# BDMstudio/audio-cut

Hardware: AMD Instinct MI355X
Metric: audio-seconds processed/sec (separate+detect) per GPU; cut-point index parity (higher is better)
Workload: dtype f32

## Files before the change

### audio_cut_amd/_native.py

```python
from __future__ import annotations

import ctypes as C
import threading
import os
from pathlib import Path
from typing import Optional, Sequence, Tuple

import numpy as np
import torch

_LIB_NAME = "libaudiocut_hip.so"
_lib: Optional[C.CDLL] = None


class NativeError(RuntimeError):
    pass


def library_path() -> Path:
    return Path(__file__).resolve().parent / os.environ.get("AUDIOCUT_HIP_LIBNAME", _LIB_NAME)


def load() -> C.CDLL:
    global _lib
    if _lib is not None:
        return _lib
    path = library_path()
    if not path.exists():
        raise NativeError(f"{path} is missing: build it with `make -C audio_cut_amd/csrc` "
                          f"(there is no CPU fallback for the HIP path)")
    lib = C.CDLL(str(path))
    _declare(lib)
    if lib.ac_abi_version() != 6:
        raise NativeError("libaudiocut_hip.so ABI version mismatch")
    if lib.ac_stereo_abi_version() != 1:
        raise NativeError("libaudiocut_hip.so stereo ABI version mismatch")
    if lib.ac_onset_abi_version() != 1:
        raise NativeError("libaudiocut_hip.so onset ABI version mismatch")
    if lib.ac_beat_abi_version() != 1:
        raise NativeError("libaudiocut_hip.so beat ABI version mismatch")
    if lib.ac_hybrid_abi_version() != 1:
        raise NativeError("libaudiocut_hip.so hybrid ABI version mismatch")
    if lib.ac_export_abi_version() != 1:
        raise NativeError("libaudiocut_hip.so export ABI version mismatch")
    if lib.ac_asr_abi_version() != 1:
        raise NativeError("libaudiocut_hip.so asr ABI version mismatch")
    if lib.ac_profile_abi_version() != 1:
        raise NativeError("libaudiocut_hip.so profile ABI version mismatch")
    if lib.ac_final_abi_version() != 1:
        raise NativeError("libaudiocut_hip.so final-layer ABI version mismatch")
    if lib.ac_load_abi_version() != 1:
        raise NativeError("libaudiocut_hip.so loader ABI version mismatch")
    if lib.ac_pack_abi_version() != 1:
        raise NativeError("libaudiocut_hip.so pack ABI version mismatch")
    _lib = lib
    return lib


_P = C.c_void_p
_I64 = C.c_int64
_I = C.c_int

SIGNATURES = {
    "ac_abi_version": (C.c_int, []),
    "ac_last_error": (C.c_char_p, []),
    "ac_ctx_create": (C.c_int, [_I, C.POINTER(_P)]),
    "ac_ctx_destroy": (C.c_int, [_P]),
    "ac_frame_rms": (C.c_int, [_P, _P, _I64, _I, _I, _I, _P, _I64, _P]),
    "ac_frame_rms_multi": (C.c_int, [_P, _P, _I64, _I, _P, _P, _P, _P, _P]),
    "ac_stft2048_features": (C.c_int, [_P, _P, _I64, _I, _P, _P, _P, _P, _P, _I64, _P]),
    "ac_onset_strength": (C.c_int, [_P, _P, _I64, _P, _I, _I, _I, _P, _P, _P]),
    "ac_tempogram_parts": (C.c_int, [_I64]),
    "ac_tempogram_reduce": (C.c_int, [_P, _P, _I64, _I, _P, _P, _P, _P, _P]),
    "ac_yin_f0": (C.c_int, [_P, _P, _I64, _I, _I, _I, _I, C.c_double, _P, _P, _I64, _P]),
    "ac_moving_meansq_db_f64": (C.c_int, [_P, _P, _I64, _I, _P, _P]),
    "ac_next_leq_scratch": (C.c_int64, [_I64]),
    "ac_next_leq_scan": (C.c_int, [_P, _P, _I64, C.c_double, _P, _P, _P]),
    "ac_window_argmin_f64": (C.c_int, [_P, _P, _I64, _P, _P, _I, _P, _P, _P]),
    "ac_zero_cross_nearest": (C.c_int, [_P, _P, _I64, _P, _I, _I, _P, _P]),
    "ac_quiet_guard_slow": (C.c_int, [_P, _P, _I64, _P, _I, _I, _I, _P, _P, _P]),
    "ac_pause_cut_points": (C.c_int, [_P, _P, _I64, _P, _P, _I, _I, _I, _P, _P, _P]),
    "ac_mdx_stft": (C.c_int, [_P, _P, _I64, _P, _P, _P, _I, _P, _P, _P]),
    "ac_mdx_istft": (C.c_int, [_P, _P, _I, _P, _P, _P]),
    "ac_mdx_assemble_ola": (C.c_int, [_P, _P, _I64, _P, _P, _P, _P, _P, _P, _I, _P, _P, _P]),
    "ac_mdx_chunk_vocal": (C.c_int, [_P, _P, _P, _P, _P, _I, _P, _P]),
    "ac_sum_squares": (C.c_int, [_P, _P, _I64, _P, _I, _P]),
    "ac_window_sum_squares": (C.c_int, [_P, _P, _I64, _P, _P, _I, _P, _P]),
    "ac_conv3x3_f16x3": (C.c_int, [_P, _P, _P, _P, _P, _I, _I, _I, _I, _I, C.c_float, _I, _P, _P, _P]),
    "ac_conv3x3_f16x3_w96": (C.c_int, [_P, _P, _P, _P, _P, _I, _I, _I, _I, _I, C.c_float, _I, _P, _P, _P]),
    "ac_conv3x3_f16x3_s8": (C.c_int, [_P, _P, _P, _P, _P, _I, _I, _I, _I, _I, C.c_float, _I, _P, _P, _P]),
    "ac_conv3x3_f16x3_first": (C.c_int, [_P, _P, _P, _P, _P, _P, _P, _I, _I, _I, _I, _I, _I, C.c_float, _I, _P, C.c_float, C.c_float,
                                         _P, _P]),
    "ac_tdf_linear_f16x3": (C.c_int, [_P, _P, _P, _P, _P, _P, _P, _I64, _I, _I, _I, _I, C.c_float, _P, _P, _P]),
    "ac_tdf_small_fused": (C.c_int, [_P, _P, _P, _P, _P, _P, _P, _P, _P, _I64, _I, _I, _I, _I, _P, _P]),
    "ac_conv1x1_small": (C.c_int, [_P, _P, _P, _P, _P, _I, _I, _I, _I64, _I, _P]),
    "ac_down2x_f16x3": (C.c_int, [_P, _P, _P, _P, _P, _I, _I, _I, _I, _I, C.c_float, _P, _P, _P]),
    "ac_up2x_f16x3": (C.c_int, [_P, _P, _P, _P, _P, _P, _I, _I, _I, _I, _I, C.c_float, _P, _P, _P]),
    "ac_pyin_observe": (C.c_int, [_P, _P, _I64, _I, _I, C.c_double, C.c_double, _I, _I, _P, _P, _P, _P, _P, C.c_double, C.c_double,
                                  _P, _P, _P, _P]),
    "ac_pyin_viterbi": (C.c_int, [_P, _P, _P, _I64, _I, _I, _P, _P, C.c_double, _P, _P, _P, _P]),
    "ac_lpc_formants": (C.c_int, [_P, _P, _I64, _I, _I, _I, C.c_float, _P, _P, _I64, _P]),
    "ac_zero_crossing_rate": (C.c_int, [_P, _P, _I64, _I, _I, _P, _I64, _P]),
    "ac_stft2048_spectral": (C.c_int, [_P, _P, _I64, _I, C.c_double, _P, _P, _I64, _P]),
    "ac_segment_frame_rms": (C.c_int, [_P, _P, _I64, _P, _P, _P, _I, _I, _I, _I, _P, _I64, _P]),
    "ac_segment_sumsq_peak": (C.c_int, [_P, _P, _I64, _P, _P, _I, _P, _P, _P]),
    "ac_local_valley_tiles": (C.c_int, [_I, _I]),
    "ac_local_valley": (C.c_int, [_P, _P, _I64, _P, _I, _I, _I, _P, _P, _P, _P, _P, _P]),
    "ac_resample_poly": (C.c_int, [_P, _P, _I64, _I, _I, _P, _I64, _I64, _P, _I64, _P]),
    "ac_pack_pcm24": (C.c_int, [_P, _P, _I64, _P, _P]),
    "ac_resample_poly_segments": (C.c_int, [_P, _P, _P, _P, _P, _P, _I, _I, _I, _P, _I64, _I64, _P, _I64, _P]),
    "ac_silero_frontend": (C.c_int, [_P, _P, _P, _I, _P, _P, _P, _P, _P, _P, _P, _P, _P, _P, _P, _P, _P]),
    "ac_silero_lstm": (C.c_int, [_P, _P, _P, _P, _I, _P, _P, _P]),
    "ac_silero_out": (C.c_int, [_P, _P, _P, C.c_float, _I, _P, _P]),
    "ac_host_beat_dp": (C.c_int, [_P, _I64, C.c_double, C.c_double, _P, _P]),
}

STEREO_SIGNATURES = {
    "ac_stereo_abi_version": (C.c_int, []),
    "ac_mdx_stft_stereo": (C.c_int, [_P, _P, _I64, _P, _P, _P, _I, _P, _P, _P]),
    "ac_mdx_assemble_ola_stereo": (C.c_int, [_P, _P, _I64, _P, _P, _P, _P, _P, _P, _I, _P, _P, _P, _P, _P]),
    "ac_mdx_chunk_vocal_stereo": (C.c_int, [_P, _P, _I64, _P, _P, _P, _P, _P, _I, _I, _P, _P]),
}


ONSET_SIGNATURES = {
    "ac_onset_abi_version": (C.c_int, []),
    "ac_bar_energy_silence": (C.c_int, [_P, _P, _I64, _P, _P, _I, C.c_double, _P, _P, _P]),
    "ac_segment_pair_energy": (C.c_int, [_P, _P, _P, _I64, _P, _P, _I, _P, _P]),
}

BEAT_SIGNATURES = {
    "ac_beat_abi_version": (C.c_int, []),
    "ac_stft2048_centroid_bandwidth": (C.c_int, [_P, _P, _I64, _I, C.c_double, _P, _P, _I64, _P]),
    "ac_bar_means3": (C.c_int, [_P, _P, _I64, _P, _P, _I64, _P, _P, _I, _P, _P]),
}

HYBRID_SIGNATURES = {
    "ac_hybrid_abi_version": (C.c_int, []),
    "ac_quiet_gate_meansq": (C.c_int, [_P, _P, _I64, _I64, _P, _I, _P, _I64, _P, _P, _P]),
}

EXPORT_SIGNATURES = {
    "ac_export_abi_version": (C.c_int, []),
    "ac_mdx_assemble_pcm24": (C.c_int, [_P, _P, _I64, _I, _P, _P, _P, _P, _P, _P, _I, _P, _P, _P, _I, _P]),
}

ASR_SIGNATURES = {
    "ac_asr_abi_version": (C.c_int, []),
    "ac_resample_poly_pcm16": (C.c_int, [_P, _P, _I64, _I, _I, _P, _I64, _I64, _P, _I64, _P]),
}

PROFILE_SIGNATURES = {
    "ac_profile_abi_version": (C.c_int, []),
    "ac_abs_peak_coverage": (C.c_int, [_P, _P, _I64, C.c_double, C.c_double, _P, _P, _P, _P]),
}
FINAL_SIGNATURES = {
    "ac_final_abi_version": (C.c_int, []),
    "ac_tdf_linear_final_f16x3": (C.c_int, [_P, _P, _P, _P, _P, _P, _P, _P, _P, _P, _I64, _I, _I, _I, _I, _I, C.c_float, _P, _P]),
}
LOAD_SIGNATURES = {
    "ac_load_abi_version": (C.c_int, []),
    "ac_decode_pcm": (C.c_int, [_P, _P, _I64, _I, _I, _I, _P, _I64, _P, _P]),
}
PACK_SIGNATURES = {
    "ac_pack_abi_version": (C.c_int, []),
    "ac_pack_width": (C.c_int, [_I]),
    "ac_pack_out_align": (C.c_int, [_I]),
    "ac_pack_pcm": (C.c_int, [_P, _P, _I64, _I, _I64, _I, _P, _P]),
    "ac_mdx_assemble_pcm": (C.c_int, [_P, _P, _I64, _I, _P, _P, _P, _P, _P, _P, _I, _I, _P, _P, _P, _I, _P]),
}
from .utils.audio_export import WAV_SUBTYPES as PACK_SUBTYPES, subtype_info as pack_subtype


PROFILE_GRID_SAMPLES = 4 * 256 * 2048


def coverage_from(peak: float, count: int, n: int) -> float:
    if int(n) == 0 or float(peak) <= 1e-9:
        return 0.0
    return max(0.0, min(1.0, int(count) / int(n)))


def _declare(lib: C.CDLL) -> None:
    for name, (res, args) in (*SIGNATURES.items(), *STEREO_SIGNATURES.items(), *ONSET_SIGNATURES.items(), *BEAT_SIGNATURES.items(),
                              *HYBRID_SIGNATURES.items(), *EXPORT_SIGNATURES.items(), *ASR_SIGNATURES.items(), *PROFILE_SIGNATURES.items(),
                              *FINAL_SIGNATURES.items(), *LOAD_SIGNATURES.items(), *PACK_SIGNATURES.items()):
        fn = getattr(lib, name)
        fn.restype = res
        fn.argtypes = args


def _check(rc: int) -> None:
    if rc != 0:
        msg = load().ac_last_error()
        raise NativeError(f"libaudiocut_hip call failed ({rc}): {msg.decode() if msg else '?'}")


def _ptr(t: Optional[torch.Tensor]) -> Optional[int]:
    if t is None:
        return None
    if not t.is_contiguous():
        raise NativeError("non-contiguous tensor passed to the HIP ABI")
    return t.data_ptr()


def _stream() -> int:
    return torch.cuda.current_stream().cuda_stream


def _packed(name: str, t: Optional[torch.Tensor], n_bytes: Optional[int]) -> None:
    if t is None or n_bytes is None:
        return
    have = t.numel() * t.element_size()
    if have != n_bytes:
        raise NativeError(f"{name}: the packed weights hold {have} bytes, the shape implies {n_bytes} (see separation/conv_pack.py)")


def _conv3x3_packed_bytes(c_in: int, c_out: int, cob: int, stage: int) -> Optional[int]:
    if c_in <= 0 or c_out <= 0 or c_in % 16 or c_out % cob:
        return None
    return (c_out // cob) * (c_in // stage) * (5 if stage == 16 else 3) * 2 * (cob // 16) * 64 * 8 * 2


def _linear_packed_bytes(n: int, k: int, bn: int) -> Optional[int]:
    if n <= 0 or k <= 0 or (bn == 0 and (n % 96 or k % 32)):
        return None
    n2 = -(-n // bn) * bn if bn else n
    return 2 * n2 * (-(-k // 32) * 32) * 2


class Context:

    def __init__(self, device: str = "cuda:0"):
        if not torch.cuda.is_available():
            raise NativeError("no HIP device visible to PyTorch: the audio-cut HIP path needs a GPU")
        self.device = torch.device(device)
        if self.device.type != "cuda":
            raise NativeError(f"device {device!r} is not a HIP device")
        self.index = self.device.index if self.device.index is not None else torch.cuda.current_device()
        self.device = torch.device("cuda", self.index)
        self.lib = load()
        handle = _P()
        with torch.cuda.device(self.index):
            _check(self.lib.ac_ctx_create(self.index, C.byref(handle)))
        self._h = handle
        self._rs_filters: dict = {}
        self._pf = threading.local()

    def close(self) -> None:
        if getattr(self, "_h", None):
            self.lib.ac_ctx_destroy(self._h)
            self._h = None

    def __del__(self):
        try:
            self.close()
        except Exception:
            pass

    SMALL_UPLOAD_BYTES = 1 << 20

    def to_device(self, arr, dtype=None) -> torch.Tensor:
        t = torch.as_tensor(np.ascontiguousarray(arr))
        if dtype is not None:
            t = t.to(dtype)
        if 0 < t.numel() * t.element_size() <= self.SMALL_UPLOAD_BYTES and not t.is_cuda:
            staged = torch.empty(t.shape, dtype=t.dtype, pin_memory=True)
            staged.copy_(t)
            return staged.to(self.device, non_blocking=True)
# ... 803 lines not shown
            raise NativeError("conv1x1_small expects a contiguous float32 NCHW tensor")
        b, c, h, w = x.shape
        w2 = weight.reshape(weight.shape[0], -1)
        if w2.shape[1] != c or not w2.is_contiguous():
            raise NativeError("conv1x1_small: weight must be [C_out, C_in(,1,1)] contiguous")
        _packed("conv1x1_small (bias)", bias, w2.shape[0] * 4)
        out = torch.empty((b, w2.shape[0], h, w), dtype=torch.float32, device=self.device)
        _check(self.lib.ac_conv1x1_small(self._h, _ptr(x), _ptr(w2), _ptr(bias), _ptr(out), b, c, w2.shape[0], h * w, int(relu), _stream()))
        return out

    def down2x_f16x3(self, x: torch.Tensor, w_packed: torch.Tensor, bias: torch.Tensor, c_out: int, w_unscale: float,
                     in_amax: Optional[torch.Tensor] = None, out_amax: Optional[torch.Tensor] = None) -> torch.Tensor:
        if x.dtype != torch.float32 or x.dim() != 4 or not x.is_contiguous():
            raise NativeError("down2x_f16x3 expects a contiguous float32 NCHW tensor")
        b, c, h, w = x.shape
        _packed("down2x_f16x3", w_packed, _linear_packed_bytes(int(c_out), 4 * c, 96))
        out = torch.empty((b, c_out, h // 2, w // 2), dtype=torch.float32, device=self.device)
        pi, po = self._amax_args(b, in_amax, out_amax, h, h // 2)
        _check(self.lib.ac_down2x_f16x3(self._h, _ptr(x), _ptr(w_packed), _ptr(bias), _ptr(out), b, c, c_out, h, w, float(w_unscale),
                                        pi, po, _stream()))
        return out

    def up2x_f16x3(self, x: torch.Tensor, w_packed: torch.Tensor, bias: torch.Tensor, c_out: int, w_unscale: float,
                   skip: Optional[torch.Tensor] = None, in_amax: Optional[torch.Tensor] = None,
                   out_amax: Optional[torch.Tensor] = None) -> torch.Tensor:
        if x.dtype != torch.float32 or x.dim() != 4 or not x.is_contiguous():
            raise NativeError("up2x_f16x3 expects a contiguous float32 NCHW tensor")
        b, c, h, w = x.shape
        _packed("up2x_f16x3", w_packed, _linear_packed_bytes(4 * int(c_out), c, 96))
        out = torch.empty((b, c_out, 2 * h, 2 * w), dtype=torch.float32, device=self.device)
        if skip is not None and (skip.shape != out.shape or not skip.is_contiguous() or skip.dtype != torch.float32):
            raise NativeError("up2x_f16x3: skip must match the output")
        pi, po = self._amax_args(b, in_amax, out_amax, h, 2 * h)
        _check(self.lib.ac_up2x_f16x3(self._h, _ptr(x), _ptr(w_packed), _ptr(bias), _ptr(skip), _ptr(out), b, c, c_out, h, w,
                                      float(w_unscale), pi, po, _stream()))
        return out

    def sum_squares_parts(self, x: torch.Tensor) -> torch.Tensor:
        self._chk_f32(x)
        hit = self._pf_take("sum_squares_parts", x)
        if hit is not None:
            return hit
        n = x.numel()
        parts = min(1024, max(1, n // 4096))
        buf = torch.empty(parts, dtype=torch.float64, device=self.device)
        _check(self.lib.ac_sum_squares(self._h, _ptr(x), n, _ptr(buf), parts, _stream()))
        return buf

    WINDOW_MEAN_SQUARE_MAX = 8191

    def window_mean_squares(self, x: torch.Tensor, starts, ends) -> np.ndarray:
        self._chk_f32(x)
        a = np.asarray(starts, dtype=np.int64); b = np.asarray(ends, dtype=np.int64)
        n = int(x.numel())
        if a.shape != b.shape or a.ndim != 1:
            raise ValueError("starts / ends must be equally long 1-D sequences")
        if a.size == 0:
            return np.zeros(0, dtype=np.float64)
        if np.any(a < 0) or np.any(b > n) or np.any(b < a) or np.any(b - a > self.WINDOW_MEAN_SQUARE_MAX):
            raise ValueError("windows must lie inside the wave and be at most WINDOW_MEAN_SQUARE_MAX samples long")
        out = torch.empty(a.size, dtype=torch.float64, device=self.device)
        a_dev, b_dev = self.to_device(a), self.to_device(b)
        _check(self.lib.ac_window_sum_squares(self._h, _ptr(x), n, _ptr(a_dev), _ptr(b_dev), int(a.size), _ptr(out), _stream()))
        sums = out.cpu().numpy()
        length = (b - a).astype(np.float64)
        return np.where(length > 0, sums / np.where(length > 0, length, 1.0), 0.0)

    def mean_square(self, x: torch.Tensor) -> float:
        self._chk_f32(x)
        n = x.numel()
        if n == 0:
            return 0.0
        return float(np.sum(self.sum_squares_parts(x).cpu().numpy())) / float(n)


def host_beat_dp(localscore: np.ndarray, period: float, tightness: float):
    lib = load()
    ls = np.ascontiguousarray(localscore, dtype=np.float64)
    n = ls.size
    back = np.empty(n, dtype=np.int64)
    cum = np.zeros(n, dtype=np.float64)
    _check(lib.ac_host_beat_dp(ls.ctypes.data, n, float(period), float(tightness), back.ctypes.data, cum.ctypes.data))
    return back, cum
```

### audio_cut_amd/csrc/ac_mdx.hip

```cpp
#include <math.h>

#include "ac_common.h"
#include "../../include/audiocut_hip_stereo.h"

#define MDX_NFFT 6144
#define MDX_M 3072
#define MDX_HOP 1024
#define MDX_T 256
#define MDX_F 3072
#define MDX_ITEM 261120
#define MDX_TRIM 3072
#define MDX_GEN 254976

__device__ inline float2 cmulf(float2 a, float2 b) { return make_float2(a.x * b.x - a.y * b.y, a.x * b.y + a.y * b.x); }

__device__ inline float2 tw3072(const float2* __restrict__ tw, int q) {
    int k = 2 * q;
    if (k >= MDX_M) { const float2 t = tw[k - MDX_M]; return make_float2(-t.x, -t.y); }
    return tw[k];
}

__device__ float2* fft3072_f32(float2* a, float2* b, const float2* __restrict__ tw) {
    int Ns = 1;
    for (int pass = 0; pass < 5; ++pass) {
        for (int j = threadIdx.x; j < MDX_M / 4; j += 256) {
            const int k = j & (Ns - 1);
            float2 v0 = a[j], v1 = a[j + MDX_M / 4], v2 = a[j + MDX_M / 2], v3 = a[j + 3 * MDX_M / 4];
            if (Ns > 1) {
                const int q = k * (MDX_M / (4 * Ns));
                v1 = cmulf(v1, tw3072(tw, q));
                v2 = cmulf(v2, tw3072(tw, 2 * q));
                v3 = cmulf(v3, tw3072(tw, 3 * q));
            }
            const float2 s02 = make_float2(v0.x + v2.x, v0.y + v2.y), d02 = make_float2(v0.x - v2.x, v0.y - v2.y);
            const float2 s13 = make_float2(v1.x + v3.x, v1.y + v3.y), d13 = make_float2(v1.x - v3.x, v1.y - v3.y);
            const int base = ((j - k) << 2) + k;
            b[base] = make_float2(s02.x + s13.x, s02.y + s13.y);
            b[base + Ns] = make_float2(d02.x + d13.y, d02.y - d13.x);
            b[base + 2 * Ns] = make_float2(s02.x - s13.x, s02.y - s13.y);
            b[base + 3 * Ns] = make_float2(d02.x - d13.y, d02.y + d13.x);
        }
        __syncthreads();
        float2* t = a; a = b; b = t;
        Ns <<= 2;
    }
    {
        const float c3 = -0.5f, s3 = -0.86602540378443864676f;
        for (int j = threadIdx.x; j < MDX_M / 3; j += 256) {
            const int k = j;
            float2 v0 = a[j], v1 = a[j + 1024], v2 = a[j + 2048];
            v1 = cmulf(v1, tw3072(tw, k));
            v2 = cmulf(v2, tw3072(tw, 2 * k));
            const float2 s = make_float2(v1.x + v2.x, v1.y + v2.y);
            const float2 d = make_float2(v1.x - v2.x, v1.y - v2.y);
            const float2 m = make_float2(v0.x + c3 * s.x, v0.y + c3 * s.y);
            const float2 r = make_float2(-s3 * d.y, s3 * d.x);
            b[k] = make_float2(v0.x + s.x, v0.y + s.y);
            b[k + 1024] = make_float2(m.x + r.x, m.y + r.y);
            b[k + 2048] = make_float2(m.x - r.x, m.y - r.y);
        }
        __syncthreads();
        float2* t = a; a = b; b = t;
    }
    return a;
}

template <int CH>
__global__ __launch_bounds__(256) void k_mdx_stft(const float* __restrict__ track, int64_t n,
                                                  const int64_t* __restrict__ chunk_start,
                                                  const int64_t* __restrict__ chunk_len,
                                                  const int32_t* __restrict__ win_index,
                                                  const float2* __restrict__ tw, const float* __restrict__ hann,
                                                  float* __restrict__ spec, float* __restrict__ spec_amax) {
    __shared__ float2 s_a[MDX_M];
    __shared__ float2 s_b[MDX_M];
    const int t = blockIdx.x;
    const int item = blockIdx.y;
    const int ch = CH == 2 ? (int)blockIdx.z : 0;
    const float* x = track + (size_t)ch * n;
    const int64_t cs = chunk_start[item];
    const int64_t cl = chunk_len[item];
    const int64_t woff = (int64_t)win_index[item] * MDX_GEN - MDX_TRIM;
    for (int m = threadIdx.x; m < MDX_M; m += 256) {
        float v[2];
#pragma unroll
        for (int h = 0; h < 2; ++h) {
            const int i = 2 * m + h;
            int jj = t * MDX_HOP - MDX_NFFT / 2 + i;
            if (jj < 0) jj = -jj;
            else if (jj >= MDX_ITEM) jj = 2 * (MDX_ITEM - 1) - jj;
            const int64_t q = woff + jj;
            const float s = (q >= 0 && q < cl) ? x[cs + q] : 0.f;
            v[h] = s * hann[i];
        }
        s_a[m] = make_float2(v[0], v[1]);
    }
    __syncthreads();
    const float2* Z = fft3072_f32(s_a, s_b, tw);
    const size_t cstride = (size_t)MDX_T * MDX_F;
    float* out = spec + (size_t)item * 4 * cstride + 2 * ch * cstride + (size_t)t * MDX_F;
    float vmax = 0.f;
    for (int k = threadIdx.x; k < MDX_F; k += 256) {
        const float2 zk = Z[k];
        const float2 zn = Z[(MDX_M - k) % MDX_M];
        const float2 e = make_float2(0.5f * (zk.x + zn.x), 0.5f * (zk.y - zn.y));
        const float2 o = make_float2(0.5f * (zk.x - zn.x), 0.5f * (zk.y + zn.y));
        const float2 wo = cmulf(tw[k], o);
        const float re = e.x + wo.y, im = e.y - wo.x;
        out[k] = re;
        out[cstride + k] = im;
        if (CH == 1) {
            out[2 * cstride + k] = re;
            out[3 * cstride + k] = im;
        }
        vmax = fmaxf(vmax, fmaxf(fabsf(re), fabsf(im)));
    }
    if (spec_amax) ac_amax_commit(vmax, spec_amax + (size_t)item * MDX_T + t);
}

extern "C" int ac_mdx_stft(ac_ctx* ctx, const float* track, int64_t n, const int64_t* chunk_start, const int64_t* chunk_len,
                           const int32_t* win_index, int n_items, float* spec_out, float* spec_amax, void* stream) {
    AC_REQUIRE(ctx && track && chunk_start && chunk_len && win_index && spec_out, "null pointer");
    AC_REQUIRE(n > 0 && n_items > 0 && n_items <= 65535, "n_items must be in [1, 65535]");
    hipLaunchKernelGGL(k_mdx_stft<1>, dim3(MDX_T, n_items), dim3(256), 0, (hipStream_t)stream, track, n, chunk_start, chunk_len,
                       win_index, ctx->tw6144, ctx->hann6144, spec_out, spec_amax);
    AC_LAUNCH_CHECK();
    return AC_OK;
}

extern "C" int ac_mdx_stft_stereo(ac_ctx* ctx, const float* track, int64_t n, const int64_t* chunk_start, const int64_t* chunk_len,
                                  const int32_t* win_index, int n_items, float* spec_out, float* spec_amax, void* stream) {
    AC_REQUIRE(ctx && track && chunk_start && chunk_len && win_index && spec_out, "null pointer");
    AC_REQUIRE(n > 0 && n_items > 0 && n_items <= 65535, "n_items must be in [1, 65535]");
    hipLaunchKernelGGL(k_mdx_stft<2>, dim3(MDX_T, n_items, 2), dim3(256), 0, (hipStream_t)stream, track, n, chunk_start, chunk_len,
                       win_index, ctx->tw6144, ctx->hann6144, spec_out, spec_amax);
    AC_LAUNCH_CHECK();
    return AC_OK;
}

__global__ __launch_bounds__(256) void k_mdx_istft_frames(const float* __restrict__ spec, const float2* __restrict__ tw,
                                                          const float* __restrict__ hann, float* __restrict__ frames) {
    __shared__ float2 s_a[MDX_M];
    __shared__ float2 s_b[MDX_M];
    const int t = blockIdx.x, ch = blockIdx.y, item = blockIdx.z;
    const size_t cstride = (size_t)MDX_T * MDX_F;
    const float* re_p = spec + ((size_t)item * 4 + 2 * ch) * cstride + (size_t)t * MDX_F;
    const float* im_p = re_p + cstride;
    for (int k = threadIdx.x; k < MDX_M; k += 256) {
        float2 xk = make_float2(re_p[k], k == 0 ? 0.f : im_p[k]);
        float2 xm = (k == 0) ? make_float2(0.f, 0.f) : make_float2(re_p[MDX_M - k], im_p[MDX_M - k]);
        const float2 e = make_float2(0.5f * (xk.x + xm.x), 0.5f * (xk.y - xm.y));
        const float2 d = make_float2(0.5f * (xk.x - xm.x), 0.5f * (xk.y + xm.y));
        const float2 w = tw[k];
        const float2 o = cmulf(make_float2(w.x, -w.y), d);
        s_a[k] = make_float2(e.x - o.y, -(e.y + o.x));
    }
    __syncthreads();
    const float2* z = fft3072_f32(s_a, s_b, tw);
    const float inv = 1.0f / (float)MDX_M;
    float* out = frames + (((size_t)item * 2 + ch) * MDX_T + t) * MDX_NFFT;
    for (int m = threadIdx.x; m < MDX_M; m += 256) {
        const float2 v = z[m];
        const float x0 = v.x * inv, x1 = -v.y * inv;
        const float2 hw = reinterpret_cast<const float2*>(hann)[m];
        reinterpret_cast<float2*>(out)[m] = make_float2(x0 * hw.x, x1 * hw.y);
    }
}

__global__ __launch_bounds__(256) void k_mdx_istft_ola(const float* __restrict__ frames, const float* __restrict__ env,
                                                       float* __restrict__ wave) {
    const int64_t idx = (int64_t)blockIdx.x * 256 + threadIdx.x;
    const int64_t row = idx / MDX_ITEM;
    const int nn = (int)(idx - row * MDX_ITEM);
    const int p = nn + MDX_NFFT / 2;
    int t_lo = (p - (MDX_NFFT - 1) + MDX_HOP - 1) / MDX_HOP;
    if (p - (MDX_NFFT - 1) <= 0) t_lo = 0;
    int t_hi = p / MDX_HOP;
    if (t_hi > MDX_T - 1) t_hi = MDX_T - 1;
    const float* base = frames + (size_t)row * MDX_T * MDX_NFFT;
    float acc = 0.f;
    for (int t = t_lo; t <= t_hi; ++t) acc += base[(size_t)t * MDX_NFFT + (p - t * MDX_HOP)];
    wave[idx] = acc / env[p];
}

extern "C" int ac_mdx_istft(ac_ctx* ctx, const float* spec, int n_items, float* wave_out, float* scratch, void* stream) {
    AC_REQUIRE(ctx && spec && wave_out && scratch, "null pointer");
    AC_REQUIRE(n_items > 0 && n_items <= 65535, "n_items must be in [1, 65535]");
    hipLaunchKernelGGL(k_mdx_istft_frames, dim3(MDX_T, 2, n_items), dim3(256), 0, (hipStream_t)stream, spec, ctx->tw6144,
                       ctx->hann6144, scratch);
    AC_LAUNCH_CHECK();
    const int64_t total = (int64_t)n_items * 2 * MDX_ITEM;
    hipLaunchKernelGGL(k_mdx_istft_ola, dim3((unsigned)(total / 256)), dim3(256), 0, (hipStream_t)stream, scratch,
                       ctx->ola_env6144, wave_out);
    AC_LAUNCH_CHECK();
    return AC_OK;
}

template <int CH>
__global__ __launch_bounds__(256) void k_mdx_assemble_ola(const float* __restrict__ track, int64_t n, const float* __restrict__ wave,
                                                          const int64_t* __restrict__ chunk_start,
                                                          const int64_t* __restrict__ chunk_len,
                                                          const int64_t* __restrict__ eff_start,
                                                          const int64_t* __restrict__ eff_end,
                                                          const int32_t* __restrict__ item_base, int n_chunks,
                                                          float* __restrict__ vocal_out, float* __restrict__ inst_out,
                                                          float* __restrict__ vocal_st_out, float* __restrict__ inst_st_out) {
    const int64_t g = (int64_t)blockIdx.x * 256 + threadIdx.x;
    if (g >= n) return;
    int lo = 0, hi = n_chunks;
    while (lo < hi) { const int mid = (lo + hi) >> 1; if (eff_end[mid] > g) hi = mid; else lo = mid + 1; }
    const int c_lo = lo;
    const float m0 = track[g];
    const float m1 = CH == 2 ? track[n + g] : m0;
    float v_acc = 0.f, i_acc = 0.f, w_acc = 0.f;
    float v0_acc = 0.f, v1_acc = 0.f, i0_acc = 0.f, i1_acc = 0.f;
    for (int c = c_lo; c < n_chunks && eff_start[c] <= g; ++c) {
        if (eff_end[c] <= g) continue;
        const int64_t q = g - chunk_start[c];
        if (q < 0 || q >= chunk_len[c]) continue;
        const int item = item_base[c] + (int)(q / MDX_GEN);
        const int pos = MDX_TRIM + (int)(q % MDX_GEN);
        const float w0 = wave[((size_t)item * 2 + 0) * MDX_ITEM + pos];
        const float w1 = wave[((size_t)item * 2 + 1) * MDX_ITEM + pos];
        const float vocal = (w0 + w1) * 0.5f;
        const float inst = ((m0 - w0) + (m1 - w1)) * 0.5f;
        v_acc += vocal;
        i_acc += inst;
        w_acc += 1.0f;
        if (CH == 2) {
            v0_acc += w0; v1_acc += w1;
            i0_acc += m0 - w0; i1_acc += m1 - w1;
        }
    }
    if (w_acc == 0.f) w_acc = 1.0f;
    vocal_out[g] = v_acc / w_acc;
    inst_out[g] = i_acc / w_acc;
    if (CH == 2) {
        if (vocal_st_out) { vocal_st_out[g] = v0_acc / w_acc; vocal_st_out[n + g] = v1_acc / w_acc; }
        if (inst_st_out) { inst_st_out[g] = i0_acc / w_acc; inst_st_out[n + g] = i1_acc / w_acc; }
    }
}

extern "C" int ac_mdx_assemble_ola(ac_ctx* ctx, const float* track, int64_t n, const float* wave, const int64_t* chunk_start,
                                   const int64_t* chunk_len, const int64_t* eff_start, const int64_t* eff_end,
                                   const int32_t* item_base, int n_chunks, float* vocal_out, float* inst_out, void* stream) {
    AC_REQUIRE(ctx && track && wave && chunk_start && chunk_len && eff_start && eff_end && item_base && vocal_out && inst_out,
               "null pointer");
    AC_REQUIRE(n > 0 && n_chunks > 0, "sizes must be positive");
    const int64_t blocks = (n + 255) / 256;
    AC_REQUIRE(blocks < (1LL << 31), "track too long");
    hipLaunchKernelGGL(k_mdx_assemble_ola<1>, dim3((unsigned)blocks), dim3(256), 0, (hipStream_t)stream, track, n, wave, chunk_start,
                       chunk_len, eff_start, eff_end, item_base, n_chunks, vocal_out, inst_out, nullptr, nullptr);
    AC_LAUNCH_CHECK();
    return AC_OK;
}

extern "C" int ac_mdx_assemble_ola_stereo(ac_ctx* ctx, const float* track, int64_t n, const float* wave, const int64_t* chunk_start,
                                          const int64_t* chunk_len, const int64_t* eff_start, const int64_t* eff_end,
                                          const int32_t* item_base, int n_chunks, float* vocal_out, float* inst_out,
                                          float* vocal_st_out, float* inst_st_out, void* stream) {
    AC_REQUIRE(ctx && track && wave && chunk_start && chunk_len && eff_start && eff_end && item_base && vocal_out && inst_out,
               "null pointer");
    AC_REQUIRE(n > 0 && n_chunks > 0, "sizes must be positive");
    const int64_t blocks = (n + 255) / 256;
    AC_REQUIRE(blocks < (1LL << 31), "track too long");
    hipLaunchKernelGGL(k_mdx_assemble_ola<2>, dim3((unsigned)blocks), dim3(256), 0, (hipStream_t)stream, track, n, wave, chunk_start,
                       chunk_len, eff_start, eff_end, item_base, n_chunks, vocal_out, inst_out, vocal_st_out, inst_st_out);
    AC_LAUNCH_CHECK();
    return AC_OK;
}

template <int CH>
__global__ __launch_bounds__(256) void k_mdx_chunk_vocal(const float* __restrict__ track, int64_t n, const float* __restrict__ wave,
                                                         const int64_t* __restrict__ chunk_start,
                                                         const int64_t* __restrict__ chunk_len,
                                                         const int64_t* __restrict__ out_offset,
// ... 75 lines not shown
```

Measured before the change: 1538.

## Replace LDS radix-4 FFT3072 with register-resident 16-point-per-thread FFT in MDX STFT/ISTFT

```diff
diff --git a/audio_cut_amd/_native.py b/audio_cut_amd/_native.py
--- a/audio_cut_amd/_native.py
+++ b/audio_cut_amd/_native.py
@@ -53,6 +53,8 @@
         raise NativeError("libaudiocut_hip.so loader ABI version mismatch")
     if lib.ac_pack_abi_version() != 1:
         raise NativeError("libaudiocut_hip.so pack ABI version mismatch")
+    if lib.ac_fft_abi_version() != 1:
+        raise NativeError("libaudiocut_hip.so fft ABI version mismatch")
     _lib = lib
     return lib
 
@@ -169,6 +171,12 @@
     "ac_pack_pcm": (C.c_int, [_P, _P, _I64, _I, _I64, _I, _P, _P]),
     "ac_mdx_assemble_pcm": (C.c_int, [_P, _P, _I64, _I, _P, _P, _P, _P, _P, _P, _I, _I, _P, _P, _P, _I, _P]),
 }
+FFT_SIGNATURES = {
+    "ac_fft_abi_version": (C.c_int, []),
+    "ac_mdx_fft3072_frames": (C.c_int, []),
+    "ac_mdx_fft3072": (C.c_int, [_P, _P, _P, _I, _P]),
+    "ac_mdx_fft3072_ref": (C.c_int, [_P, _P, _P, _I, _P]),
+}
 from .utils.audio_export import WAV_SUBTYPES as PACK_SUBTYPES, subtype_info as pack_subtype
 
 
@@ -184,7 +192,7 @@
 def _declare(lib: C.CDLL) -> None:
     for name, (res, args) in (*SIGNATURES.items(), *STEREO_SIGNATURES.items(), *ONSET_SIGNATURES.items(), *BEAT_SIGNATURES.items(),
                               *HYBRID_SIGNATURES.items(), *EXPORT_SIGNATURES.items(), *ASR_SIGNATURES.items(), *PROFILE_SIGNATURES.items(),
-                              *FINAL_SIGNATURES.items(), *LOAD_SIGNATURES.items(), *PACK_SIGNATURES.items()):
+                              *FINAL_SIGNATURES.items(), *LOAD_SIGNATURES.items(), *PACK_SIGNATURES.items(), *FFT_SIGNATURES.items()):
         fn = getattr(lib, name)
         fn.restype = res
         fn.argtypes = args
@@ -1154,3 +1162,16 @@
     cum = np.zeros(n, dtype=np.float64)
     _check(lib.ac_host_beat_dp(ls.ctypes.data, n, float(period), float(tightness), back.ctypes.data, cum.ctypes.data))
     return back, cum
+
+
+def mdx_fft3072_frames() -> int:
+    return int(load().ac_mdx_fft3072_frames())
+
+
+def mdx_fft3072(ctx: Context, x: torch.Tensor, reference: bool = False) -> torch.Tensor:
+    if x.dtype != torch.float32 or x.device != ctx.device or x.dim() != 3 or tuple(x.shape[1:]) != (3072, 2):
+        raise NativeError("mdx_fft3072 expects float32 [n, 3072, 2] on the context's device")
+    out = torch.empty_like(x, memory_format=torch.contiguous_format)
+    fn = ctx.lib.ac_mdx_fft3072_ref if reference else ctx.lib.ac_mdx_fft3072
+    _check(fn(ctx._h, _ptr(x), _ptr(out), x.shape[0], _stream()))
+    return out
diff --git a/audio_cut_amd/csrc/ac_fft3072.h b/audio_cut_amd/csrc/ac_fft3072.h
--- /dev/null
+++ b/audio_cut_amd/csrc/ac_fft3072.h
@@ -0,0 +1,197 @@
+#ifndef AC_FFT3072_H
+#define AC_FFT3072_H
+
+#include <hip/hip_runtime.h>
+
+#define MDX_M 3072
+
+__device__ inline float2 cmulf(float2 a, float2 b) { return make_float2(a.x * b.x - a.y * b.y, a.x * b.y + a.y * b.x); }
+
+__device__ inline float2 tw3072(const float2* __restrict__ tw, int q) {
+    int k = 2 * q;
+    if (k >= MDX_M) { const float2 t = tw[k - MDX_M]; return make_float2(-t.x, -t.y); }
+    return tw[k];
+}
+
+__device__ float2* fft3072_f32(float2* a, float2* b, const float2* __restrict__ tw) {
+    int Ns = 1;
+    for (int pass = 0; pass < 5; ++pass) {
+        for (int j = threadIdx.x; j < MDX_M / 4; j += 256) {
+            const int k = j & (Ns - 1);
+            float2 v0 = a[j], v1 = a[j + MDX_M / 4], v2 = a[j + MDX_M / 2], v3 = a[j + 3 * MDX_M / 4];
+            if (Ns > 1) {
+                const int q = k * (MDX_M / (4 * Ns));
+                v1 = cmulf(v1, tw3072(tw, q));
+                v2 = cmulf(v2, tw3072(tw, 2 * q));
+                v3 = cmulf(v3, tw3072(tw, 3 * q));
+            }
+            const float2 s02 = make_float2(v0.x + v2.x, v0.y + v2.y), d02 = make_float2(v0.x - v2.x, v0.y - v2.y);
+            const float2 s13 = make_float2(v1.x + v3.x, v1.y + v3.y), d13 = make_float2(v1.x - v3.x, v1.y - v3.y);
+            const int base = ((j - k) << 2) + k;
+            b[base] = make_float2(s02.x + s13.x, s02.y + s13.y);
+            b[base + Ns] = make_float2(d02.x + d13.y, d02.y - d13.x);
+            b[base + 2 * Ns] = make_float2(s02.x - s13.x, s02.y - s13.y);
+            b[base + 3 * Ns] = make_float2(d02.x - d13.y, d02.y + d13.x);
+        }
+        __syncthreads();
+        float2* t = a; a = b; b = t;
+        Ns <<= 2;
+    }
+    {
+        const float c3 = -0.5f, s3 = -0.86602540378443864676f;
+        for (int j = threadIdx.x; j < MDX_M / 3; j += 256) {
+            const int k = j;
+            float2 v0 = a[j], v1 = a[j + 1024], v2 = a[j + 2048];
+            v1 = cmulf(v1, tw3072(tw, k));
+            v2 = cmulf(v2, tw3072(tw, 2 * k));
+            const float2 s = make_float2(v1.x + v2.x, v1.y + v2.y);
+            const float2 d = make_float2(v1.x - v2.x, v1.y - v2.y);
+            const float2 m = make_float2(v0.x + c3 * s.x, v0.y + c3 * s.y);
+            const float2 r = make_float2(-s3 * d.y, s3 * d.x);
+            b[k] = make_float2(v0.x + s.x, v0.y + s.y);
+            b[k + 1024] = make_float2(m.x + r.x, m.y + r.y);
+            b[k + 2048] = make_float2(m.x - r.x, m.y - r.y);
+        }
+        __syncthreads();
+        float2* t = a; a = b; b = t;
+    }
+    return a;
+}
+
+#ifndef FFT3072_FRAMES
+#define FFT3072_FRAMES 1
+#endif
+#define FFT3072_LDS (MDX_M + MDX_M / 16)
+__device__ __forceinline__ int fft3072_at(int p) { return p + (p >> 4); }
+__device__ __forceinline__ int fft3072_at16(int at_q, int c) { return at_q + c + (c >> 4); }
+
+__device__ __forceinline__ int fft3072_zero() { int z = 0; asm volatile("" : "+s"(z)); return z; }
+
+__device__ __forceinline__ float2 fft3072_value(float2 t) { asm volatile("" : "+v"(t.x), "+v"(t.y)); return t; }
+
+__device__ __forceinline__ void fft3072_tw_a(const float2* __restrict__ tw, float2 (&t)[12]) {
+#pragma unroll
+    for (int m = 0; m < 4; ++m)
+#pragma unroll
+        for (int mm = 1; mm < 4; ++mm) t[3 * m + mm - 1] = fft3072_value(tw3072(tw, 192 * m * mm));
+}
+__device__ __forceinline__ void fft3072_tw_b(const float2* __restrict__ tw, float2 (&t0)[3], float2 (&t1)[12]) {
+    const int k = threadIdx.x & 15;
+#pragma unroll
+    for (int mm = 1; mm < 4; ++mm) t0[mm - 1] = fft3072_value(tw3072(tw, k * 48 * mm));
+#pragma unroll
+    for (int m = 0; m < 4; ++m)
+#pragma unroll
+        for (int mm = 1; mm < 4; ++mm) t1[3 * m + mm - 1] = fft3072_value(tw3072(tw, (16 * m + k) * 12 * mm));
+}
+__device__ __forceinline__ void fft3072_tw_c(const float2* __restrict__ tw, float2 (&t0)[3], float2 (&t1)[8]) {
+    const int k = threadIdx.x;
+#pragma unroll
+    for (int mm = 1; mm < 4; ++mm) t0[mm - 1] = fft3072_value(tw3072(tw, k * 3 * mm));
+#pragma unroll
+    for (int m = 0; m < 4; ++m) {
+        t1[2 * m] = fft3072_value(tw3072(tw, k + 256 * m));
+        t1[2 * m + 1] = fft3072_value(tw3072(tw, 2 * (k + 256 * m)));
+    }
+}
+
+__device__ __forceinline__ float fft3072_add(float a, float b) {
+    float r;
+    asm("v_add_f32_e32 %0, %1, %2" : "=v"(r) : "v"(a), "v"(b));
+    return r;
+}
+
+__device__ __forceinline__ float2 fft3072_cmul(float2 a, float2 b) {
+    return make_float2(a.x * b.x - a.y * b.y, fft3072_add(a.y * b.x, a.x * b.y));
+}
+
+__device__ __forceinline__ void fft3072_r4(float2 v0, float2 v1, float2 v2, float2 v3, float2& o0, float2& o1, float2& o2, float2& o3) {
+    const float2 s02 = make_float2(fft3072_add(v0.x, v2.x), fft3072_add(v0.y, v2.y)), d02 = make_float2(v0.x - v2.x, v0.y - v2.y);
+    const float2 s13 = make_float2(fft3072_add(v3.x, v1.x), fft3072_add(v3.y, v1.y)), d13 = make_float2(v1.x - v3.x, v1.y - v3.y);
+    o0 = make_float2(fft3072_add(s02.x, s13.x), fft3072_add(s02.y, s13.y));
+    o1 = make_float2(fft3072_add(d02.x, d13.y), d02.y - d13.x);
+    o2 = make_float2(s02.x - s13.x, s02.y - s13.y);
+    o3 = make_float2(d02.x - d13.y, fft3072_add(d02.y, d13.x));
+}
+
+template <bool FIRST>
+__device__ __forceinline__ void fft3072_r4x2(float2 (&v)[16], const float2 (&t0)[3], const float2 (&t1)[12]) {
+    float2 u[4][4];
+#pragma unroll
+    for (int b = 0; b < 4; ++b) {
+        float2 v0 = v[b], v1 = v[b + 4], v2 = v[b + 8], v3 = v[b + 12];
+        if (!FIRST) {
+            v1 = fft3072_cmul(v1, t0[0]);
+            v2 = fft3072_cmul(v2, t0[1]);
+            v3 = fft3072_cmul(v3, t0[2]);
+        }
+        fft3072_r4(v0, v1, v2, v3, u[b][0], u[b][1], u[b][2], u[b][3]);
+    }
+#pragma unroll
+    for (int m = 0; m < 4; ++m) {
+        const float2 v0 = u[0][m];
+        const float2 v1 = fft3072_cmul(u[1][m], t1[3 * m]);
+        const float2 v2 = fft3072_cmul(u[2][m], t1[3 * m + 1]);
+        const float2 v3 = fft3072_cmul(u[3][m], t1[3 * m + 2]);
+        fft3072_r4(v0, v1, v2, v3, v[m], v[m + 4], v[m + 8], v[m + 12]);
+    }
+}
+
+template <class Fill>
+__device__ __forceinline__ void fft3072_regs(Fill fill, float2* __restrict__ x, float2* __restrict__ y, const float2* __restrict__ tw,
+                                             int rot, float2 (&z)[12]) {
+    const int tid = threadIdx.x;
+    const int idle = rot & 3, wave = tid >> 6;
+    const bool active = wave != idle;
+    const int j0 = tid - (wave > idle ? 64 : 0);
+    float2 tb0[3], tb1[12], tc0[3], tc1[8];
+    if (active) {
+        float2 v[16], ta[12];
+        fill(j0, v);
+        fft3072_tw_a(tw, ta);
+        fft3072_r4x2<true>(v, tb0, ta);
+#pragma unroll
+        for (int i = 0; i < 16; ++i) x[17 * j0 + i] = v[i];
+        fft3072_tw_b(tw + fft3072_zero(), tb0, tb1);
+    }
+    __syncthreads();
+    if (active) {
+        float2 v[16];
+#pragma unroll
+        for (int i = 0; i < 16; ++i) v[i] = x[fft3072_at16(fft3072_at(j0), 192 * i)];
+        fft3072_r4x2<false>(v, tb0, tb1);
+        const int base = fft3072_at(256 * (j0 >> 4) + (j0 & 15));
+#pragma unroll
+        for (int i = 0; i < 16; ++i) y[fft3072_at16(base, 16 * i)] = v[i];
+    }
+    fft3072_tw_c(tw + fft3072_zero(), tc0, tc1);
+    __syncthreads();
+    {
+        float2 u[3][4];
+        const int at = fft3072_at(tid);
+#pragma unroll
+        for (int g = 0; g < 3; ++g) {
+            const float2 v0 = y[fft3072_at16(at, 256 * g)];
+            const float2 v1 = fft3072_cmul(y[fft3072_at16(at, 256 * g + 768)], tc0[0]);
+            const float2 v2 = fft3072_cmul(y[fft3072_at16(at, 256 * g + 1536)], tc0[1]);
+            const float2 v3 = fft3072_cmul(y[fft3072_at16(at, 256 * g + 2304)], tc0[2]);
+            fft3072_r4(v0, v1, v2, v3, u[g][0], u[g][1], u[g][2], u[g][3]);
+        }
+        const float c3 = -0.5f, s3 = -0.86602540378443864676f;
+#pragma unroll
+        for (int m = 0; m < 4; ++m) {
+            const float2 v0 = u[0][m];
+            const float2 v1 = fft3072_cmul(u[1][m], tc1[2 * m]);
+            const float2 v2 = fft3072_cmul(u[2][m], tc1[2 * m + 1]);
+            const float2 s = make_float2(fft3072_add(v1.x, v2.x), fft3072_add(v1.y, v2.y));
+            const float2 d = make_float2(v1.x - v2.x, v1.y - v2.y);
+            const float2 mid = make_float2(v0.x + c3 * s.x, v0.y + c3 * s.y);
+            const float2 r = make_float2(-s3 * d.y, s3 * d.x);
+            z[m] = make_float2(fft3072_add(v0.x, s.x), fft3072_add(v0.y, s.y));
+            z[m + 4] = make_float2(fft3072_add(r.x, mid.x), fft3072_add(r.y, mid.y));
+            z[m + 8] = make_float2(mid.x - r.x, mid.y - r.y);
+        }
+    }
+}
+
+#endif
diff --git a/audio_cut_amd/csrc/ac_mdx.hip b/audio_cut_amd/csrc/ac_mdx.hip
--- a/audio_cut_amd/csrc/ac_mdx.hip
+++ b/audio_cut_amd/csrc/ac_mdx.hip
@@ -1,10 +1,11 @@
 #include <math.h>
 
 #include "ac_common.h"
+#include "ac_fft3072.h"
+#include "../../include/audiocut_hip_fft.h"
 #include "../../include/audiocut_hip_stereo.h"
 
 #define MDX_NFFT 6144
-#define MDX_M 3072
 #define MDX_HOP 1024
 #define MDX_T 256
 #define MDX_F 3072
@@ -12,117 +13,91 @@
 #define MDX_TRIM 3072
 #define MDX_GEN 254976
 
-__device__ inline float2 cmulf(float2 a, float2 b) { return make_float2(a.x * b.x - a.y * b.y, a.x * b.y + a.y * b.x); }
-
-__device__ inline float2 tw3072(const float2* __restrict__ tw, int q) {
-    int k = 2 * q;
-    if (k >= MDX_M) { const float2 t = tw[k - MDX_M]; return make_float2(-t.x, -t.y); }
-    return tw[k];
-}
-
-__device__ float2* fft3072_f32(float2* a, float2* b, const float2* __restrict__ tw) {
-    int Ns = 1;
-    for (int pass = 0; pass < 5; ++pass) {
-        for (int j = threadIdx.x; j < MDX_M / 4; j += 256) {
-            const int k = j & (Ns - 1);
-            float2 v0 = a[j], v1 = a[j + MDX_M / 4], v2 = a[j + MDX_M / 2], v3 = a[j + 3 * MDX_M / 4];
-            if (Ns > 1) {
-                const int q = k * (MDX_M / (4 * Ns));
-                v1 = cmulf(v1, tw3072(tw, q));
-                v2 = cmulf(v2, tw3072(tw, 2 * q));
-                v3 = cmulf(v3, tw3072(tw, 3 * q));
-            }
-            const float2 s02 = make_float2(v0.x + v2.x, v0.y + v2.y), d02 = make_float2(v0.x - v2.x, v0.y - v2.y);
-            const float2 s13 = make_float2(v1.x + v3.x, v1.y + v3.y), d13 = make_float2(v1.x - v3.x, v1.y - v3.y);
-            const int base = ((j - k) << 2) + k;
-            b[base] = make_float2(s02.x + s13.x, s02.y + s13.y);
-            b[base + Ns] = make_float2(d02.x + d13.y, d02.y - d13.x);
-            b[base + 2 * Ns] = make_float2(s02.x - s13.x, s02.y - s13.y);
-            b[base + 3 * Ns] = make_float2(d02.x - d13.y, d02.y + d13.x);
-        }
-        __syncthreads();
-        float2* t = a; a = b; b = t;
-        Ns <<= 2;
-    }
-    {
-        const float c3 = -0.5f, s3 = -0.86602540378443864676f;
-        for (int j = threadIdx.x; j < MDX_M / 3; j += 256) {
-            const int k = j;
-            float2 v0 = a[j], v1 = a[j + 1024], v2 = a[j + 2048];
-            v1 = cmulf(v1, tw3072(tw, k));
-            v2 = cmulf(v2, tw3072(tw, 2 * k));
-            const float2 s = make_float2(v1.x + v2.x, v1.y + v2.y);
-            const float2 d = make_float2(v1.x - v2.x, v1.y - v2.y);
-            const float2 m = make_float2(v0.x + c3 * s.x, v0.y + c3 * s.y);
-            const float2 r = make_float2(-s3 * d.y, s3 * d.x);
-            b[k] = make_float2(v0.x + s.x, v0.y + s.y);
-            b[k + 1024] = make_float2(m.x + r.x, m.y + r.y);
-            b[k + 2048] = make_float2(m.x - r.x, m.y - r.y);
-        }
-        __syncthreads();
-        float2* t = a; a = b; b = t;
-    }
-    return a;
-}
-
 template <int CH>
-__global__ __launch_bounds__(256) void k_mdx_stft(const float* __restrict__ track, int64_t n,
+__global__ __launch_bounds__(256, 3) void k_mdx_stft(const float* __restrict__ track, int64_t n,
                                                   const int64_t* __restrict__ chunk_start,
                                                   const int64_t* __restrict__ chunk_len,
                                                   const int32_t* __restrict__ win_index,
                                                   const float2* __restrict__ tw, const float* __restrict__ hann,
                                                   float* __restrict__ spec, float* __restrict__ spec_amax) {
-    __shared__ float2 s_a[MDX_M];
-    __shared__ float2 s_b[MDX_M];
-    const int t = blockIdx.x;
+    __shared__ float2 s_a[FFT3072_LDS];
+    __shared__ float2 s_b[FFT3072_LDS];
     const int item = blockIdx.y;
     const int ch = CH == 2 ? (int)blockIdx.z : 0;
     const float* x = track + (size_t)ch * n;
     const int64_t cs = chunk_start[item];
     const int64_t cl = chunk_len[item];
     const int64_t woff = (int64_t)win_index[item] * MDX_GEN - MDX_TRIM;
-    for (int m = threadIdx.x; m < MDX_M; m += 256) {
-        float v[2];
-#pragma unroll
-        for (int h = 0; h < 2; ++h) {
-            const int i = 2 * m + h;
-            int jj = t * MDX_HOP - MDX_NFFT / 2 + i;
-            if (jj < 0) jj = -jj;
-            else if (jj >= MDX_ITEM) jj = 2 * (MDX_ITEM - 1) - jj;
-            const int64_t q = woff + jj;
-            const float s = (q >= 0 && q < cl) ? x[cs + q] : 0.f;
-            v[h] = s * hann[i];
+    const size_t cstride = (size_t)MDX_T * MDX_F;
+    float2 *sx = s_a, *sy = s_b;
+#pragma unroll 1
+    for (int f = 0; f < FFT3072_FRAMES; ++f) {
+        const int t = blockIdx.x * FFT3072_FRAMES + f;
+        const int zf = fft3072_zero();
+        const float2* twf = tw + zf;
+        const float2* hann2 = reinterpret_cast<const float2*>(hann) + zf;
+        const int j_lo = t * MDX_HOP - MDX_NFFT / 2;
+        const bool inside = j_lo >= 0 && j_lo + MDX_NFFT <= MDX_ITEM && woff + j_lo >= 0 && woff + j_lo + MDX_NFFT <= cl;
+        float2 z[12];
+        fft3072_regs([&](int j0, float2 (&v)[16]) {
+            if (inside) {
+                const float* xf = x + cs + woff + j_lo;
+#pragma unroll
+                for (int p = 0; p < 16; ++p) {
+                    const int m = j0 + 192 * p;
+                    const float2 hw = hann2[m];
+                    v[p] = make_float2(xf[2 * m] * hw.x, xf[2 * m + 1] * hw.y);
+                }
+                return;
+            }
+#pragma unroll
+            for (int p = 0; p < 16; ++p) {
+                const int m = j0 + 192 * p;
+                const float2 hw = hann2[m];
+                float s[2];
+#pragma unroll
+                for (int h = 0; h < 2; ++h) {
+                    int jj = j_lo + 2 * m + h;
+                    if (jj < 0) jj = -jj;
+                    else if (jj >= MDX_ITEM) jj = 2 * (MDX_ITEM - 1) - jj;
+                    const int64_t q = woff + jj;
+                    s[h] = (q >= 0 && q < cl) ? x[cs + q] : 0.f;
+                }
+                v[p] = make_float2(s[0] * hw.x, s[1] * hw.y);
+            }
+        }, sx, sy, twf, t, z);
+#pragma unroll
+        for (int i = 0; i < 12; ++i) sx[fft3072_at16(fft3072_at(threadIdx.x), 256 * i)] = z[i];
+        __syncthreads();
+        float* out = spec + (size_t)item * 4 * cstride + 2 * ch * cstride + (size_t)t * MDX_F;
+        float vmax = 0.f;
+#pragma unroll
+        for (int i = 0; i < 12; ++i) {
+            const int k = threadIdx.x + 256 * i;
+            const float2 zk = z[i];
+            const float2 zn = sx[fft3072_at((MDX_M - k) % MDX_M)];
+            const float2 e = make_float2(0.5f * (zk.x + zn.x), 0.5f * (zk.y - zn.y));
+            const float2 o = make_float2(0.5f * (zk.x - zn.x), 0.5f * (zk.y + zn.y));
+            const float2 wo = cmulf(twf[k], o);
+            const float re = e.x + wo.y, im = e.y - wo.x;
+            out[k] = re;
+            out[cstride + k] = im;
+            if (CH == 1) {
+                out[2 * cstride + k] = re;
+                out[3 * cstride + k] = im;
+            }
+            vmax = fmaxf(vmax, fmaxf(fabsf(re), fabsf(im)));
         }
-        s_a[m] = make_float2(v[0], v[1]);
-    }
-    __syncthreads();
-    const float2* Z = fft3072_f32(s_a, s_b, tw);
-    const size_t cstride = (size_t)MDX_T * MDX_F;
-    float* out = spec + (size_t)item * 4 * cstride + 2 * ch * cstride + (size_t)t * MDX_F;
-    float vmax = 0.f;
-    for (int k = threadIdx.x; k < MDX_F; k += 256) {
-        const float2 zk = Z[k];
-        const float2 zn = Z[(MDX_M - k) % MDX_M];
-        const float2 e = make_float2(0.5f * (zk.x + zn.x), 0.5f * (zk.y - zn.y));
-        const float2 o = make_float2(0.5f * (zk.x - zn.x), 0.5f * (zk.y + zn.y));
-        const float2 wo = cmulf(tw[k], o);
-        const float re = e.x + wo.y, im = e.y - wo.x;
-        out[k] = re;
-        out[cstride + k] = im;
-        if (CH == 1) {
-            out[2 * cstride + k] = re;
-            out[3 * cstride + k] = im;
-        }
-        vmax = fmaxf(vmax, fmaxf(fabsf(re), fabsf(im)));
-    }
-    if (spec_amax) ac_amax_commit(vmax, spec_amax + (size_t)item * MDX_T + t);
+        if (spec_amax) ac_amax_commit(vmax, spec_amax + (size_t)item * MDX_T + t);
+        float2* sw = sx; sx = sy; sy = sw;
+    }
 }
 
 extern "C" int ac_mdx_stft(ac_ctx* ctx, const float* track, int64_t n, const int64_t* chunk_start, const int64_t* chunk_len,
                            const int32_t* win_index, int n_items, float* spec_out, float* spec_amax, void* stream) {
     AC_REQUIRE(ctx && track && chunk_start && chunk_len && win_index && spec_out, "null pointer");
     AC_REQUIRE(n > 0 && n_items > 0 && n_items <= 65535, "n_items must be in [1, 65535]");
-    hipLaunchKernelGGL(k_mdx_stft<1>, dim3(MDX_T, n_items), dim3(256), 0, (hipStream_t)stream, track, n, chunk_start, chunk_len,
+    hipLaunchKernelGGL(k_mdx_stft<1>, dim3(MDX_T / FFT3072_FRAMES, n_items), dim3(256), 0, (hipStream_t)stream, track, n, chunk_start, chunk_len,
                        win_index, ctx->tw6144, ctx->hann6144, spec_out, spec_amax);
     AC_LAUNCH_CHECK();
     return AC_OK;
@@ -132,38 +107,49 @@
                                   const int32_t* win_index, int n_items, float* spec_out, float* spec_amax, void* stream) {
     AC_REQUIRE(ctx && track && chunk_start && chunk_len && win_index && spec_out, "null pointer");
     AC_REQUIRE(n > 0 && n_items > 0 && n_items <= 65535, "n_items must be in [1, 65535]");
-    hipLaunchKernelGGL(k_mdx_stft<2>, dim3(MDX_T, n_items, 2), dim3(256), 0, (hipStream_t)stream, track, n, chunk_start, chunk_len,
+    hipLaunchKernelGGL(k_mdx_stft<2>, dim3(MDX_T / FFT3072_FRAMES, n_items, 2), dim3(256), 0, (hipStream_t)stream, track, n, chunk_start, chunk_len,
                        win_index, ctx->tw6144, ctx->hann6144, spec_out, spec_amax);
     AC_LAUNCH_CHECK();
     return AC_OK;
 }
 
-__global__ __launch_bounds__(256) void k_mdx_istft_frames(const float* __restrict__ spec, const float2* __restrict__ tw,
+__global__ __launch_bounds__(256, 3) void k_mdx_istft_frames(const float* __restrict__ spec, const float2* __restrict__ tw,
                                                           const float* __restrict__ hann, float* __restrict__ frames) {
-    __shared__ float2 s_a[MDX_M];
-    __shared__ float2 s_b[MDX_M];
-    const int t = blockIdx.x, ch = blockIdx.y, item = blockIdx.z;
+    __shared__ float2 s_a[FFT3072_LDS];
+    __shared__ float2 s_b[FFT3072_LDS];
+    const int ch = blockIdx.y, item = blockIdx.z;
     const size_t cstride = (size_t)MDX_T * MDX_F;
-    const float* re_p = spec + ((size_t)item * 4 + 2 * ch) * cstride + (size_t)t * MDX_F;
-    const float* im_p = re_p + cstride;
-    for (int k = threadIdx.x; k < MDX_M; k += 256) {
-        float2 xk = make_float2(re_p[k], k == 0 ? 0.f : im_p[k]);
-        float2 xm = (k == 0) ? make_float2(0.f, 0.f) : make_float2(re_p[MDX_M - k], im_p[MDX_M - k]);
-        const float2 e = make_float2(0.5f * (xk.x + xm.x), 0.5f * (xk.y - xm.y));
-        const float2 d = make_float2(0.5f * (xk.x - xm.x), 0.5f * (xk.y + xm.y));
-        const float2 w = tw[k];
-        const float2 o = cmulf(make_float2(w.x, -w.y), d);
-        s_a[k] = make_float2(e.x - o.y, -(e.y + o.x));
-    }
-    __syncthreads();
-    const float2* z = fft3072_f32(s_a, s_b, tw);
-    const float inv = 1.0f / (float)MDX_M;
-    float* out = frames + (((size_t)item * 2 + ch) * MDX_T + t) * MDX_NFFT;
-    for (int m = threadIdx.x; m < MDX_M; m += 256) {
-        const float2 v = z[m];
-        const float x0 = v.x * inv, x1 = -v.y * inv;
-        const float2 hw = reinterpret_cast<const float2*>(hann)[m];
-        reinterpret_cast<float2*>(out)[m] = make_float2(x0 * hw.x, x1 * hw.y);
+#pragma unroll 1
+    for (int f = 0; f < FFT3072_FRAMES; ++f) {
+        const int t = blockIdx.x * FFT3072_FRAMES + f;
+        const float* re_p = spec + ((size_t)item * 4 + 2 * ch) * cstride + (size_t)t * MDX_F;
+        const float* im_p = re_p + cstride;
+        const int zf = fft3072_zero();
+        const float2* twf = tw + zf;
+        const float* hannf = hann + zf;
+        float2 z[12];
+        fft3072_regs([&](int j0, float2 (&v)[16]) {
+#pragma unroll
+            for (int p = 0; p < 16; ++p) {
+                const int k = j0 + 192 * p;
+                float2 xk = make_float2(re_p[k], k == 0 ? 0.f : im_p[k]);
+                float2 xm = (k == 0) ? make_float2(0.f, 0.f) : make_float2(re_p[MDX_M - k], im_p[MDX_M - k]);
+                const float2 e = make_float2(0.5f * (xk.x + xm.x), 0.5f * (xk.y - xm.y));
+                const float2 d = make_float2(0.5f * (xk.x - xm.x), 0.5f * (xk.y + xm.y));
+                const float2 wk = twf[k];
+                const float2 o = cmulf(make_float2(wk.x, -wk.y), d);
+                v[p] = make_float2(e.x - o.y, -(e.y + o.x));
+            }
+        }, s_a, s_b, twf, t, z);
+        const float inv = 1.0f / (float)MDX_M;
+        float* out = frames + (((size_t)item * 2 + ch) * MDX_T + t) * MDX_NFFT;
+#pragma unroll
+        for (int i = 0; i < 12; ++i) {
+            const float2 v = z[i];
+            const float x0 = v.x * inv, x1 = -v.y * inv;
+            const float2 hw = reinterpret_cast<const float2*>(hannf)[threadIdx.x + 256 * i];
+            reinterpret_cast<float2*>(out)[threadIdx.x + 256 * i] = make_float2(x0 * hw.x, x1 * hw.y);
+        }
     }
 }
 
@@ -186,12 +172,64 @@
 extern "C" int ac_mdx_istft(ac_ctx* ctx, const float* spec, int n_items, float* wave_out, float* scratch, void* stream) {
     AC_REQUIRE(ctx && spec && wave_out && scratch, "null pointer");
     AC_REQUIRE(n_items > 0 && n_items <= 65535, "n_items must be in [1, 65535]");
-    hipLaunchKernelGGL(k_mdx_istft_frames, dim3(MDX_T, 2, n_items), dim3(256), 0, (hipStream_t)stream, spec, ctx->tw6144,
+    hipLaunchKernelGGL(k_mdx_istft_frames, dim3(MDX_T / FFT3072_FRAMES, 2, n_items), dim3(256), 0, (hipStream_t)stream, spec, ctx->tw6144,
                        ctx->hann6144, scratch);
     AC_LAUNCH_CHECK();
     const int64_t total = (int64_t)n_items * 2 * MDX_ITEM;
     hipLaunchKernelGGL(k_mdx_istft_ola, dim3((unsigned)(total / 256)), dim3(256), 0, (hipStream_t)stream, scratch,
                        ctx->ola_env6144, wave_out);
+    AC_LAUNCH_CHECK();
+    return AC_OK;
+}
+
+__global__ __launch_bounds__(256, 3) void k_fft3072(const float2* __restrict__ in, float2* __restrict__ out, int n,
+                                                 const float2* __restrict__ tw) {
+    __shared__ float2 s_a[FFT3072_LDS];
+    __shared__ float2 s_b[FFT3072_LDS];
+#pragma unroll 1
+    for (int f = 0; f < FFT3072_FRAMES; ++f) {
+        const int64_t t = (int64_t)blockIdx.x * FFT3072_FRAMES + f;
+        if (t >= n) break;
+        const float2* src = in + t * MDX_M;
+        float2 z[12];
+        fft3072_regs([&](int j0, float2 (&v)[16]) {
+#pragma unroll
+            for (int p = 0; p < 16; ++p) v[p] = src[j0 + 192 * p];
+        }, s_a, s_b, tw + fft3072_zero(), (int)t, z);
+#pragma unroll
+        for (int i = 0; i < 12; ++i) out[t * MDX_M + threadIdx.x + 256 * i] = z[i];
+    }
+}
+
+__global__ __launch_bounds__(256) void k_fft3072_ref(const float2* __restrict__ in, float2* __restrict__ out,
+                                                     const float2* __restrict__ tw) {
+    __shared__ float2 s_a[MDX_M];
+    __shared__ float2 s_b[MDX_M];
+    const size_t base = (size_t)blockIdx.x * MDX_M;
+    for (int m = threadIdx.x; m < MDX_M; m += 256) s_a[m] = in[base + m];
+    __syncthreads();
+    const float2* z = fft3072_f32(s_a, s_b, tw);
+    for (int m = threadIdx.x; m < MDX_M; m += 256) out[base + m] = z[m];
+}
+
+extern "C" int ac_fft_abi_version(void) { return AC_FFT_ABI_VERSION; }
+
+extern "C" int ac_mdx_fft3072_frames(void) { return FFT3072_FRAMES; }
+
+extern "C" int ac_mdx_fft3072(ac_ctx* ctx, const float* in, float* out, int n, void* stream) {
+    AC_REQUIRE(ctx && in && out, "null pointer");
+    AC_REQUIRE(n > 0 && n <= (1 << 20), "n must be in [1, 2^20]");
+    hipLaunchKernelGGL(k_fft3072, dim3((unsigned)((n + FFT3072_FRAMES - 1) / FFT3072_FRAMES)), dim3(256), 0, (hipStream_t)stream,
+                       reinterpret_cast<const float2*>(in), reinterpret_cast<float2*>(out), n, ctx->tw6144);
+    AC_LAUNCH_CHECK();
+    return AC_OK;
+}
+
+extern "C" int ac_mdx_fft3072_ref(ac_ctx* ctx, const float* in, float* out, int n, void* stream) {
+    AC_REQUIRE(ctx && in && out, "null pointer");
+    AC_REQUIRE(n > 0 && n <= (1 << 20), "n must be in [1, 2^20]");
+    hipLaunchKernelGGL(k_fft3072_ref, dim3((unsigned)n), dim3(256), 0, (hipStream_t)stream, reinterpret_cast<const float2*>(in),
+                       reinterpret_cast<float2*>(out), ctx->tw6144);
     AC_LAUNCH_CHECK();
     return AC_OK;
 }
diff --git a/include/audiocut_hip_fft.h b/include/audiocut_hip_fft.h
--- /dev/null
+++ b/include/audiocut_hip_fft.h
@@ -0,0 +1,24 @@
+#ifndef AUDIOCUT_HIP_FFT_H
+#define AUDIOCUT_HIP_FFT_H
+
+#include "audiocut_hip.h"
+
+#ifdef __cplusplus
+extern "C" {
+#endif
+
+#define AC_FFT_ABI_VERSION 1
+
+int ac_fft_abi_version(void);
+
+int ac_mdx_fft3072_frames(void);
+
+int ac_mdx_fft3072(ac_ctx* ctx, const float* in, float* out, int n, void* stream);
+
+int ac_mdx_fft3072_ref(ac_ctx* ctx, const float* in, float* out, int n, void* stream);
+
+#ifdef __cplusplus
+}
+#endif
+
+#endif
```

Result: no change. 1548, median of 6 (+0.7%).
